# nextpyp/spr_pick

Measured on AMD Instinct MI355X. Metric: train_patches_per_sec, higher is better.
Workload: dtype f32; 1 GPU; BASELINE configs[1]: ssdn --noise_style gaussian --noise_value var, joint mode, 64x64 patches from 4 synthetic 1024x1024 micrographs, batch 32 per GPU, alpha 0.75, tau 0.01, Adam; fp32 MFMA convolutions (Winograd F(2x2,3x3) for the wide 3x3 layers); per_gpu_batch=32, global_batch=32, patch=64, parallelism=single GPU

## Files before the change

### include/sprk.h

```cpp
#ifndef SPRK_H
#define SPRK_H

#include <stddef.h>
#include <stdint.h>

#ifdef __cplusplus
extern "C" {
#endif

#define SPRK_OK 0
#define SPRK_EINVAL (-1)
#define SPRK_EWORKSPACE (-2)
#define SPRK_ELAUNCH (-3)

#define SPRK_ACT_NONE 0
#define SPRK_ACT_LEAKY 1
#define SPRK_ACT_RELU 2

typedef struct sprk_conv_geom {
    int32_t N, C1, C2, Hin, Win, up1;
    int32_t Cout, Hout, Wout;
    int32_t KH, KW, stride, dil, pad_top, pad_left;
    int32_t dtype;
} sprk_conv_geom;

#define SPRK_DT_F32 0
#define SPRK_DT_BF16 1
#define SPRK_DT_F16 2
#define SPRK_DT_MASK 0xff
#define SPRK_DT_FORCE 0x100
#define SPRK_DT_NAIVE 0x200
#define SPRK_DT_PIN 0x400
#define SPRK_DT_X16 0x8000
#define SPRK_DT_Y16 0x10000
#define SPRK_IO2(a, b) ((a) | ((b) << 4))
#define SPRK_IO3(a, b, c) ((a) | ((b) << 4) | ((c) << 8))

typedef struct sprk_conv_epilogue {
    const float *bias, *scale, *shift, *res;
    int32_t res_h, res_w, res_off;
    int32_t act;
    int32_t up2;
} sprk_conv_epilogue;

#define SPRK_ABI_VERSION 430
const char *sprk_last_error(void);
int sprk_version(void);
size_t sprk_struct_bytes(int which);
long sprk_launch_count(void);
long sprk_wino_launch_count(void);
long sprk_mask1x1_launch_count(void);
long sprk_conv16_launch_count(void);
long sprk_wgrad16_launch_count(void);

size_t sprk_conv2d_fwd_ws_bytes(const sprk_conv_geom *g);
int sprk_conv2d_fwd(const float *x, const float *x2, const float *w, float *y,
                    const sprk_conv_geom *g, const sprk_conv_epilogue *ep,
                    void *ws, size_t ws_bytes, void *stream);
size_t sprk_conv2d_bwd_data_ws_bytes(const sprk_conv_geom *g);
int sprk_conv2d_bwd_data(const float *gy, const float *w, float *gin, const sprk_conv_geom *g,
                         void *ws, size_t ws_bytes, void *stream);
size_t sprk_head1x1_fwd_ws_bytes(int K0, int N1);
int sprk_head1x1_fwd(const float *f, const float *w1, const float *b1, const float *w2, const float *b2,
                     const float *w3, const float *b3, float *out, int B, int K0, int N1, int N3, long HW, void *ws,
                     size_t ws_bytes, void *stream);

int sprk_head1x1_unrot_fwd(const float *d, const float *w1, const float *b1, const float *w2, const float *b2,
                           const float *w3, const float *b3, float *out, int B, int C, int P, int N3, void *ws,
                           size_t ws_bytes, void *stream);

int sprk_conv2d_bwd_data_masked(const float *gy, const float *w, float *gin, const sprk_conv_geom *g,
                                const float *mask_y, int mask_act, void *ws, size_t ws_bytes, void *stream);
int sprk_conv2d_bwd_data_mask_fused(const sprk_conv_geom *g);
int sprk_conv2d_storage16(const sprk_conv_geom *g, const sprk_conv_epilogue *ep);
size_t sprk_conv2d_bwd_weight_ws_bytes(const sprk_conv_geom *g);
int sprk_conv2d_bwd_weight(const float *x, const float *x2, const float *gy, float *gw,
                           const sprk_conv_geom *g, void *ws, size_t ws_bytes, void *stream);
#define SPRK_VARIANT_INTS 24
#define SPRK_STAGE_NONE (-2)
#define SPRK_STAGE_REFUSED (-1)
#define SPRK_STAGE_DIRECT 0
#define SPRK_STAGE_STEM 1
#define SPRK_STAGE_16BIT 2
#define SPRK_STAGE_WINOGRAD 3
#define SPRK_STAGE_MASK1X1 4
#define SPRK_STAGE_MFMA 5
int sprk_conv2d_variant(int which, const sprk_conv_geom *g, const sprk_conv_epilogue *ep, const void *x, const void *x2,
                        const void *y_or_gy, int32_t *out);
int sprk_conv2d_last_variant(int which, int32_t *out);

#define SPRK_DT_WPREP 0x800
#define SPRK_DT_WPREP_KIND(kind) (((kind) & 7) << 12)
#define SPRK_DT_WPREP_KIND_OF(dtype) (((dtype) >> 12) & 7)
typedef struct sprk_wprep_item {
    const float *w;
    void *dst;
    int32_t kind, blocks;
    int32_t p[12];
} sprk_wprep_item;
int sprk_conv2d_fwd_wprep(const float *w, const sprk_conv_geom *g, const sprk_conv_epilogue *ep, void *ws,
                          size_t ws_bytes, sprk_wprep_item *item);
int sprk_conv2d_bwd_data_wprep(const float *w, const sprk_conv_geom *g, void *ws, size_t ws_bytes, sprk_wprep_item *item);
int sprk_prepare_weights(const sprk_wprep_item *items, int n, void *stream);

size_t sprk_act_bwd_ws_bytes(int N, int C, int HW);
int sprk_act_bwd(const void *gy, const void *y, void *gpre, float *gbias, int act,
                 int N, int C, int H, int W, int up2, long g_image_stride, int io,
                 void *ws, size_t ws_bytes, void *stream);
#define SPRK_RED_NONE 0
#define SPRK_RED_ROWS 1
#define SPRK_RED_COLS 2
#define SPRK_RED_WGRAD 3
typedef struct sprk_reduce_item {
    const float *src;
    float *dst;
    int kind, parts, n, K, Cout, CoutP;
} sprk_reduce_item;
int sprk_conv2d_bwd_weight_partial(const float *x, const float *x2, const float *gy, float *gw,
                                   const sprk_conv_geom *g, void *ws, size_t ws_bytes,
                                   sprk_reduce_item *item, void *stream);
int sprk_act_bwd_partial(const void *gy, const void *y, void *gpre, float *gbias, int act,
                         int N, int C, int H, int W, int up2, long g_image_stride, int io,
                         void *ws, size_t ws_bytes, sprk_reduce_item *item, void *stream);
int sprk_reduce_items(const sprk_reduce_item *items, int n, void *stream);

int sprk_concat_up_bwd(const float *gin, float *ga, float *gb, int N, int C1, int C2, int H, int W,
                       int up1, void *stream);

int sprk_shift_maxpool2_fwd(const void *x, void *y, int NC, int H, int W, int shift, int io, void *stream);
int sprk_shift_maxpool2_bwd(const void *gy, const void *x, void *gx, int NC, int H, int W, int shift, int act,
                            int io, void *stream);
int sprk_rot4_stack_fwd(const float *x, float *y, int B, int C, int P, void *stream);
int sprk_rot4_stack_bwd(const float *gy, float *gx, int B, int C, int P, void *stream);
int sprk_unrot4_shift_concat_fwd(const void *d, void *f, int B, int C, int P, int io, void *stream);
int sprk_unrot4_shift_concat_bwd(const void *gf, void *gd, int B, int C, int P, int io, void *stream);
int sprk_unrot_act_bwd_eligible(int B, int C, int P, int act);
int sprk_conv2d_fwd_unrot_eligible(const sprk_conv_geom *g, const sprk_conv_epilogue *ep);
int sprk_conv2d_fwd_unrot(const float *x, const float *x2, const float *w, float *f, const sprk_conv_geom *g,
                          const sprk_conv_epilogue *ep, void *ws, size_t ws_bytes, void *stream);
// ... 105 lines not shown
```

### spr_pick_amd/_lib.py

```python
import ctypes
import os

_HERE = os.path.dirname(os.path.abspath(__file__))
LIB_PATH = os.environ.get("SPRK_LIB") or os.path.join(_HERE, "libsprk.so")

ACT_NONE, ACT_LEAKY, ACT_RELU = 0, 1, 2
DT_F32, DT_BF16, DT_F16 = 0, 1, 2
DT_NAIVE = 0x200
DT_WPREP = 0x800
DT_X16, DT_Y16 = 0x8000, 0x10000
DT_PIN = 0x400
DT_FORCE = 0x100
DTYPES = {"f32": DT_F32, "fp32": DT_F32, "bf16": DT_BF16, "f16": DT_F16, "fp16": DT_F16,
          "bf16!": DT_BF16 | DT_FORCE, "f16!": DT_F16 | DT_FORCE}

c_f = ctypes.c_void_p
c_i = ctypes.c_int
c_vp = ctypes.c_void_p
c_sz = ctypes.c_size_t


class ConvGeom(ctypes.Structure):
    _fields_ = [(n, ctypes.c_int32) for n in
                ("N", "C1", "C2", "Hin", "Win", "up1", "Cout", "Hout", "Wout",
                 "KH", "KW", "stride", "dil", "pad_top", "pad_left", "dtype")]


class ConvEpilogue(ctypes.Structure):
    _fields_ = [("bias", c_vp), ("scale", c_vp), ("shift", c_vp), ("res", c_vp),
                ("res_h", ctypes.c_int32), ("res_w", ctypes.c_int32), ("res_off", ctypes.c_int32),
                ("act", ctypes.c_int32), ("up2", ctypes.c_int32)]


class AdamItem(ctypes.Structure):
    _fields_ = [("p", c_vp), ("g", c_vp), ("m", c_vp), ("v", c_vp), ("n", ctypes.c_long)]


class ReduceItem(ctypes.Structure):
    _fields_ = [("src", c_vp), ("dst", c_vp), ("kind", ctypes.c_int32), ("parts", ctypes.c_int32), ("n", ctypes.c_int32),
                ("K", ctypes.c_int32), ("Cout", ctypes.c_int32), ("CoutP", ctypes.c_int32)]


class WprepItem(ctypes.Structure):
    _fields_ = [("w", c_vp), ("dst", c_vp), ("kind", ctypes.c_int32), ("blocks", ctypes.c_int32), ("p", ctypes.c_int32 * 12)]


_SIGS = {
    "sprk_last_error": (ctypes.c_char_p, []),
    "sprk_version": (c_i, []),
    "sprk_struct_bytes": (c_sz, [c_i]),
    "sprk_launch_count": (ctypes.c_long, []),
    "sprk_wino_launch_count": (ctypes.c_long, []),
    "sprk_mask1x1_launch_count": (ctypes.c_long, []),
    "sprk_conv16_launch_count": (ctypes.c_long, []),
    "sprk_wgrad16_launch_count": (ctypes.c_long, []),
    "sprk_conv2d_fwd_ws_bytes": (c_sz, [ctypes.POINTER(ConvGeom)]),
    "sprk_conv2d_fwd": (c_i, [c_f, c_f, c_f, c_f, ctypes.POINTER(ConvGeom), ctypes.POINTER(ConvEpilogue), c_vp, c_sz, c_vp]),
    "sprk_conv2d_fwd_wprep": (c_i, [c_f, ctypes.POINTER(ConvGeom), ctypes.POINTER(ConvEpilogue), c_vp, c_sz, ctypes.POINTER(WprepItem)]),
    "sprk_conv2d_bwd_data_wprep": (c_i, [c_f, ctypes.POINTER(ConvGeom), c_vp, c_sz, ctypes.POINTER(WprepItem)]),
    "sprk_prepare_weights": (c_i, [ctypes.POINTER(WprepItem), c_i, c_vp]),
    "sprk_head1x1_fwd_ws_bytes": (c_sz, [c_i, c_i]),
    "sprk_head1x1_fwd": (c_i, [c_f, c_f, c_f, c_f, c_f, c_f, c_f, c_f, c_i, c_i, c_i, c_i, ctypes.c_long, c_vp, c_sz, c_vp]),
    "sprk_head1x1_unrot_fwd": (c_i, [c_f, c_f, c_f, c_f, c_f, c_f, c_f, c_f, c_i, c_i, c_i, c_i, c_vp, c_sz, c_vp]),
    "sprk_conv2d_bwd_data_ws_bytes": (c_sz, [ctypes.POINTER(ConvGeom)]),
    "sprk_conv2d_bwd_data": (c_i, [c_f, c_f, c_f, ctypes.POINTER(ConvGeom), c_vp, c_sz, c_vp]),
    "sprk_conv2d_bwd_data_masked": (c_i, [c_f, c_f, c_f, ctypes.POINTER(ConvGeom), c_f, c_i, c_vp, c_sz, c_vp]),
    "sprk_conv2d_bwd_weight_ws_bytes": (c_sz, [ctypes.POINTER(ConvGeom)]),
    "sprk_conv2d_storage16": (c_i, [ctypes.POINTER(ConvGeom), ctypes.POINTER(ConvEpilogue)]),
    "sprk_conv2d_bwd_weight": (c_i, [c_f, c_f, c_f, c_f, ctypes.POINTER(ConvGeom), c_vp, c_sz, c_vp]),
    "sprk_conv2d_bwd_weight_partial": (c_i, [c_f, c_f, c_f, c_f, ctypes.POINTER(ConvGeom), c_vp, c_sz, ctypes.POINTER(ReduceItem), c_vp]),
    "sprk_act_bwd_partial": (c_i, [c_f, c_f, c_f, c_f, c_i, c_i, c_i, c_i, c_i, c_i, ctypes.c_long, c_i, c_vp, c_sz, ctypes.POINTER(ReduceItem), c_vp]),
    "sprk_reduce_items": (c_i, [ctypes.POINTER(ReduceItem), c_i, c_vp]),
    "sprk_act_bwd_ws_bytes": (c_sz, [c_i, c_i, c_i]),
    "sprk_act_bwd": (c_i, [c_f, c_f, c_f, c_f, c_i, c_i, c_i, c_i, c_i, c_i, ctypes.c_long, c_i, c_vp, c_sz, c_vp]),
    "sprk_concat_up_bwd": (c_i, [c_f, c_f, c_f, c_i, c_i, c_i, c_i, c_i, c_i, c_vp]),
    "sprk_shift_maxpool2_fwd": (c_i, [c_f, c_f, c_i, c_i, c_i, c_i, c_i, c_vp]),
    "sprk_shift_maxpool2_bwd": (c_i, [c_f, c_f, c_f, c_i, c_i, c_i, c_i, c_i, c_i, c_vp]),
    "sprk_rot4_stack_fwd": (c_i, [c_f, c_f, c_i, c_i, c_i, c_vp]),
    "sprk_rot4_stack_bwd": (c_i, [c_f, c_f, c_i, c_i, c_i, c_vp]),
    "sprk_unrot4_shift_concat_fwd": (c_i, [c_f, c_f, c_i, c_i, c_i, c_i, c_vp]),
    "sprk_unrot4_shift_concat_bwd": (c_i, [c_f, c_f, c_i, c_i, c_i, c_i, c_vp]),
    "sprk_unrot_act_bwd_eligible": (c_i, [c_i, c_i, c_i, c_i]),
    "sprk_conv2d_fwd_unrot_eligible": (c_i, [ctypes.POINTER(ConvGeom), ctypes.POINTER(ConvEpilogue)]),
    "sprk_conv2d_bwd_data_mask_fused": (c_i, [ctypes.POINTER(ConvGeom)]),
    "sprk_conv2d_variant": (c_i, [c_i, ctypes.POINTER(ConvGeom), ctypes.POINTER(ConvEpilogue), c_vp, c_vp, c_vp,
                                  ctypes.POINTER(ctypes.c_int32)]),
    "sprk_conv2d_last_variant": (c_i, [c_i, ctypes.POINTER(ctypes.c_int32)]),
    "sprk_conv2d_fwd_unrot": (c_i, [c_f, c_f, c_f, c_f, ctypes.POINTER(ConvGeom), ctypes.POINTER(ConvEpilogue), c_vp, c_sz, c_vp]),
    "sprk_unrot_act_bwd": (c_i, [c_f, c_f, c_f, c_f, c_i, c_i, c_i, c_i, c_vp, c_sz, ctypes.POINTER(ReduceItem), c_vp]),
    "sprk_bn_ws_bytes": (c_sz, [c_i, c_i, c_i, c_i]),
    "sprk_bn_train_fwd": (c_i, [c_f, c_f, c_f, c_f, c_f, c_f, c_f, c_f, c_i, c_i, c_i, c_i, ctypes.c_float, ctypes.c_float, c_i, c_vp, c_sz, c_vp]),
    "sprk_bn_eval_fwd": (c_i, [c_f, c_f, c_f, c_f, c_f, c_f, c_i, c_i, c_i, ctypes.c_float, c_i, c_vp]),
    "sprk_bn_train_bwd": (c_i, [c_f, c_f, c_f, c_f, c_f, c_f, c_f, c_f, c_f, c_i, c_i, c_i, c_i, c_i, c_vp, c_sz, c_vp]),
    "sprk_crop_add_fwd": (c_i, [c_f, c_f, c_f, ctypes.c_long, c_i, c_i, c_i, c_i, c_i, c_i, c_vp]),
    "sprk_crop_embed_bwd": (c_i, [c_f, c_f, ctypes.c_long, c_i, c_i, c_i, c_i, c_i, c_i, c_vp]),
    "sprk_noise_std_fwd": (c_i, [c_f, c_f, c_f, c_i, c_i, c_vp]),
    "sprk_noise_std_bwd": (c_i, [c_f, c_f, c_f, c_i, c_i, c_vp]),
    "sprk_joint_loss_fwd": (c_i, [c_f, c_f, c_f, c_f, c_f, c_f, c_i, c_i, c_i, c_i, ctypes.c_float, ctypes.c_float, c_vp]),
    "sprk_joint_loss_bwd": (c_i, [c_f, c_f, c_f, c_f, c_f, c_f, c_f, c_i, c_i, c_i, c_i, ctypes.c_float, ctypes.c_float, c_vp]),
    "sprk_reparam_fwd": (c_i, [c_f, c_f, c_f, c_i, c_i, c_vp]),
    "sprk_reparam_bwd": (c_i, [c_f, c_f, c_f, c_f, c_i, c_i, c_vp]),
    "sprk_adam_multi": (c_i, [c_vp, c_vp, c_i, c_i, c_f, c_f, c_f, ctypes.c_float, ctypes.c_float, ctypes.c_float, c_vp]),
    "sprk_adam_multi_skip": (c_i, [c_vp, c_vp, c_i, c_i, c_f, c_f, c_f, ctypes.c_float, ctypes.c_float, ctypes.c_float, c_vp, c_vp]),
    "sprk_unscale_check": (c_i, [c_f, ctypes.c_long, c_f, c_vp, c_vp]),
    "sprk_loss_scale_update": (c_i, [c_f, c_f, c_vp, c_vp, c_vp, c_vp, ctypes.c_float, ctypes.c_float, c_i, c_vp]),
    "sprk_pu_loss": (c_i, [c_f, c_f, c_f, c_i, ctypes.c_float, c_f, c_f, c_vp]),
# ... 63 lines not shown
```

### spr_pick_amd/csrc/conv.hip

```cpp
#include "common.h"
#include "conv16.h"
#include "mask1x1.h"
#include "wgrad16.h"
#include "wino.h"
#include "wprep_dev.h"

#include <cstdlib>

#include "conv_dev.h"
#include "io_dev.h"


namespace {

inline bool naive_of(const sprk_conv_geom *g) { return (g->dtype & SPRK_DT_NAIVE) != 0; }

constexpr int kZeroFloats = 256;
__device__ __attribute__((aligned(64))) float g_zero_block[kZeroFloats];

__device__ __forceinline__ void stage_planes(float *dst, const float *base, long imgStride, long cs, int nch, int N,
                                             int Hin, int Win, int Ws, int up, int vec, const float *zeros,
                                             const PlaneGeom &g, int n0, int iy0, int ixa, int lw, int lane) {
    const int imgElems = g.inRows * g.pitch;
    const int planeElems = g.NI * imgElems;
    const int per = vec ? 256 : 64;
    const int nGroups = (planeElems + per - 1) / per;
    const int nw = g.nw;
    const int gstart = g.deal ? 0 : lw, gstep = g.deal ? 1 : nw, cstep = g.deal ? nw : 1;
    for (int gi = gstart; gi < nGroups; gi += gstep) {
        const int e = vec ? gi * 256 + lane * 4 : gi * 64 + lane;
        const int il = fast_div(e, g.invImg);
        const int rem = e - il * imgElems;
        const int r = fast_div(rem, g.invPitch);
        const int j = rem - r * g.pitch;
        const int n = n0 + il, iy = iy0 + r, ix = ixa + j;
        const bool inb = e < planeElems;
        const bool ok = inb && n < N && (unsigned)iy < (unsigned)Hin && (unsigned)ix < (unsigned)Win;
        const int cl0 = g.deal ? (lw + nw - (gi % nw)) % nw : 0;
        const float *p = base + (long)n * imgStride + (up ? (long)(iy >> 1) * Ws + (ix >> 1) : (long)iy * Ws + ix) +
                         (long)cl0 * cs;
        long step = (long)cstep * cs;
        if (!ok) {
            p = zeros + lane * 4;
            step = 0;
        }
        float *d = dst + gi * per + cl0 * g.cplane;
        for (int cl = cl0; cl < nch; cl += cstep) {
            if (inb) {
                if (vec)
                    dma16(p, d);
                else
                    dma4(p, d);
            }
            p += step;
// ... 1427 lines not shown
#endif

int sprk_conv2d_storage16(const sprk_conv_geom *g, const sprk_conv_epilogue *ep) {
    if (!g || check_geom(g) != SPRK_OK) return 0;
    const int dt = g->dtype & SPRK_DT_MASK;
    if ((dt != SPRK_DT_BF16 && dt != SPRK_DT_F16) || naive_of(g) || g->stride != 1) return 0;
    sprk_conv_geom q = *g;
    q.dtype = (g->dtype & ~(SPRK_DT_WPREP | SPRK_DT_WPREP_KIND(7))) | SPRK_DT_X16 | SPRK_DT_Y16;
    int r = 0;
    if (sprk::conv16_kind(sprk::Corr(q, ep)) >= 2) r |= 1;
    if (sprk::conv16_kind(sprk::Corr(q)) >= 2) r |= 2;
    if (sprk::wgrad16_eligible(q)) r |= 4;
    return r;
}

static size_t corr_ws_bytes(const sprk::Corr &c) {
    FwdPlan p;
    if (!plan_fwd(c, &p)) return 0;
    size_t need = p.wsBytes;
    if (sprk::wino_eligible(c)) need = std::max(need, sprk::wino_ws_bytes(c));
    if (c.dt() != SPRK_DT_F32) need = std::max(need, sprk::conv16_ws_bytes(c));
    return need;
}

size_t sprk_conv2d_fwd_ws_bytes(const sprk_conv_geom *g) {
    if (!g) return 0;
    size_t need = 0;
    for (int v = 0; v < 4; ++v) {
        sprk_conv_epilogue e = sprk::kNoEpilogue;
        e.up2 = v & 1;
        e.res = (v & 2) ? (const float *)g : nullptr;
        need = std::max(need, corr_ws_bytes(sprk::Corr(*g, &e)));
    }
    return need;
}

size_t sprk_conv2d_bwd_data_ws_bytes(const sprk_conv_geom *g) {
    return (g && g->stride == 1) ? corr_ws_bytes(sprk::Corr(*g)) : 0;
}

static int mask_in_place(float *gin, const float *mask_y, int mask_act, const sprk_conv_geom *g, hipStream_t s) {
    const int t = (g->dtype & SPRK_DT_Y16) ? (g->dtype & SPRK_DT_MASK) : 0;
    return sprk_act_bwd(gin, mask_y, gin, nullptr, mask_act, g->N, g->C1 + g->C2, g->Hin, g->Win, 0, 0, SPRK_IO3(t, t, t),
                        nullptr, 0, s);
}

static bool mask1x1_takes(const sprk_conv_geom *g, const sprk::Corr &c, const FwdPlan &p) {
    return g->KH == 1 && g->KW == 1 && g->stride == 1 && g->dil == 1 && g->pad_top == 0 && g->pad_left == 0 && !g->up1 &&
           g->C2 == 0 && g->Hin == g->Hout && g->Win == g->Wout && c.dt() == SPRK_DT_F32 && !c.x16() && !c.y16() &&
           ((long)g->Hin * g->Win) % 4 == 0 && (long)g->Hin * g->Win < (1L << 30) && p.MT >= 2 &&
           sprk::mask1x1_steps(g->Cout, p.CK) > 0;
}

static FwdVariant fwd_route(bool bwd, const sprk_conv_geom *g, const sprk_conv_epilogue *ep, const void *x, const void *x2,
                            const void *y, const void *mask_y, FwdPlan *p, bool unrot = false) {
    FwdVariant v{};
    if (naive_of(g) || (bwd && g->stride != 1)) {
        StemPlan sp;
        v.stage = (bwd && !naive_of(g) && plan_stem_bwd(g, &sp)) ? SPRK_STAGE_STEM : SPRK_STAGE_DIRECT;
        return v;
    }
    const sprk::Corr c = bwd ? sprk::Corr(*g) : sprk::Corr(*g, ep);
    if (c.dt() != SPRK_DT_F32 && sprk::conv16_eligible(c)) {
        v.stage = SPRK_STAGE_16BIT;
    } else if (c.dtype & (SPRK_DT_X16 | SPRK_DT_Y16)) {
        v.stage = SPRK_STAGE_REFUSED;
    } else if (sprk::wino_eligible(c)) {
        v.stage = SPRK_STAGE_WINOGRAD;
        v.wino = sprk::wino_variant(c, mask_y != nullptr, unrot ? g->N / 4 : 0);
    } else if (!plan_fwd(c, p)) {
        v.stage = SPRK_STAGE_REFUSED;
    } else {
        v = fwd_variant(c, *p, x, x2, y);
        v.stage = (bwd && mask_y && mask1x1_takes(g, c, *p) && aligned16(x) && aligned16(y) && aligned16(mask_y))
                      ? SPRK_STAGE_MASK1X1
                      : SPRK_STAGE_MFMA;
    }
    return v;
}

static int conv_dispatch(bool bwd, const float *x, const float *x2, const float *w, float *y, const sprk_conv_geom *g,
                         const sprk_conv_epilogue *ep, const float *mask_y, int mask_act, void *ws, size_t ws_bytes,
                         void *stream, bool unrot = false) {
    const char *who = bwd ? "conv2d_bwd_data" : unrot ? "conv2d_fwd_unrot" : "conv2d_fwd";
    if (int rc = check_geom(g)) return rc;
    SPRK_REQUIRE(!unrot || sprk_conv2d_fwd_unrot_eligible(g, ep), "conv2d_fwd_unrot: no kernel with an un-rotated store for this layer");
    SPRK_REQUIRE(x && w && y, "%s: null tensor", who);
    if (bwd) {
        SPRK_REQUIRE(mask_act == SPRK_ACT_NONE || (mask_y && !g->up1), "conv2d_bwd_data: mask needs the saved input, no upsampling");
        if (mask_act == SPRK_ACT_NONE) mask_y = nullptr;
    } else {
        SPRK_REQUIRE(g->C2 == 0 || x2, "conv2d_fwd: C2 > 0 but x2 is null");
        SPRK_REQUIRE(!ep || !ep->scale || ep->shift, "conv2d_fwd: scale without shift");
    }
    hipStream_t s = (hipStream_t)stream;
    auto masked = [&](int rc) { return (rc || !mask_y) ? rc : mask_in_place(y, mask_y, mask_act, g, s); };

    FwdPlan p;
    const FwdVariant v = fwd_route(bwd, g, ep, x, x2, y, mask_y, &p, unrot);
    if (!sprk::wprep_describing()) t_last_fwd[bwd ? 1 : 0] = v;

    if (v.stage == SPRK_STAGE_DIRECT || v.stage == SPRK_STAGE_STEM) {
        if (sprk::wprep_describing()) return SPRK_OK;
        if (bwd) {
            DirectArgs a{nullptr, nullptr, w, x, y, *g, sprk::kNoEpilogue};
            StemPlan sp;
            if (v.stage == SPRK_STAGE_STEM && plan_stem_bwd(g, &sp)) {
                hipLaunchKernelGGL(conv_bwd_data_stem_kernel, dim3(g->N * sp.tilesX * sp.tilesY), dim3(kStemTW * kStemTH),
                                   sp.ldsBytes, s, a, sp.wr, sp.wc, sp.tilesX, sp.tilesY);
                return masked(sprk::check_launch("conv_bwd_data_stem"));
            }
            const long total = (long)g->N * (g->C1 + g->C2) * g->Hin * g->Win;
            hipLaunchKernelGGL(conv_bwd_data_direct_kernel, dim3(sprk::ew_blocks(total)), dim3(256), 0, s, a);
            return masked(sprk::check_launch("conv_bwd_data_direct"));
        }
        DirectArgs a{x, x2, w, nullptr, y, *g, ep ? *ep : sprk::kNoEpilogue};
        const long total = (long)g->N * g->Cout * g->Hout * g->Wout;
        hipLaunchKernelGGL(conv_fwd_direct_kernel, dim3(sprk::ew_blocks(total)), dim3(256), 0, s, a);
        return sprk::check_launch("conv_fwd_direct");
    }
    const sprk::Corr c = bwd ? sprk::Corr(*g) : sprk::Corr(*g, ep);

    if (v.stage == SPRK_STAGE_16BIT) return masked(sprk::conv16_run(c, x, x2, w, y, ws, ws_bytes, s));
    if (int rc = check_storage32(who, c.dtype)) return rc;

    if (v.stage == SPRK_STAGE_WINOGRAD) {
        if (int rc = sprk::check_ws(who, ws, ws_bytes, sprk::wino_ws_bytes(c))) return rc;
        if (int rc = sprk::wino_conv(c, v.wino, x, x2, w, y, (float *)ws, mask_y, mask_act, s)) return rc;
        return sprk::check_launch(bwd ? "wino_conv(bwd_data)" : "wino_conv");
    }
    SPRK_REQUIRE(!unrot, "conv2d_fwd_unrot: the call left the Winograd stage");

    SPRK_REQUIRE(v.stage != SPRK_STAGE_REFUSED, "%s: geometry does not fit LDS", who);
    if (int rc = sprk::check_ws(who, ws, ws_bytes, p.wsBytes)) return rc;
    float *wsf = (float *)ws;
    if (int rc = transform_weights(w, wsf, g->Cout, g->C1 + g->C2, g->KH * g->KW, c.taps, p, s)) return rc;
    if (v.stage == SPRK_STAGE_MASK1X1) {
        const sprk::Mask1x1Call m{x, wsf + kZeroFloats, mask_y, y, g->N, g->Cout, g->C1, g->Hin * g->Win,
                                  p.CK, p.R4, p.rows, p.ldw, p.NT, p.nblkN, mask_act};
        if (int rc = sprk::mask1x1_run(m, s)) return rc;
        return sprk::check_launch("mask1x1(bwd_data)");
    }
    const ConvArgs a = conv_args(c, p, v, x, x2, wsf, y);
    const int kclass = (v.MT == 4 && v.NT == 6) ? 0 : 2;
    sprk::prof_begin(kclass, c.flops, s);
    if (int rc = launch_fwd(a, p, v, s)) return rc;
    sprk::prof_end(kclass, s);
    return masked(sprk::check_launch(bwd ? "conv_mfma(bwd_data)" : "conv_mfma"));
}

int sprk_conv2d_fwd(const float *x, const float *x2, const float *w, float *y, const sprk_conv_geom *g,
                    const sprk_conv_epilogue *ep, void *ws, size_t ws_bytes, void *stream) {
    sprk::WprepScope scope(nullptr, g ? g->dtype : 0);
    return scope.verify(conv_dispatch(false, x, x2, w, y, g, ep, nullptr, SPRK_ACT_NONE, ws, ws_bytes, stream));
}

int sprk_conv2d_fwd_unrot_eligible(const sprk_conv_geom *g, const sprk_conv_epilogue *ep) {
    if (!g || check_geom(g) || naive_of(g)) return 0;
    const sprk::Corr c(*g, ep);
    if (c.dt() != SPRK_DT_F32 || c.x16() || c.y16()) return 0;
    return sprk::wino_unrot_eligible(c) ? 1 : 0;
}

int sprk_conv2d_fwd_unrot(const float *x, const float *x2, const float *w, float *f, const sprk_conv_geom *g,
                          const sprk_conv_epilogue *ep, void *ws, size_t ws_bytes, void *stream) {
    sprk::WprepScope scope(nullptr, g ? g->dtype : 0);
    return scope.verify(conv_dispatch(false, x, x2, w, f, g, ep, nullptr, SPRK_ACT_NONE, ws, ws_bytes, stream, true));
}

int sprk_conv2d_fwd_wprep(const float *w, const sprk_conv_geom *g, const sprk_conv_epilogue *ep, void *ws,
                          size_t ws_bytes, sprk_wprep_item *item) {
    SPRK_REQUIRE(item && w && ws, "conv2d_fwd_wprep: null argument");
    *item = sprk_wprep_item{};
    sprk::WprepScope scope(item, 0);
    const float *dummy = (const float *)ws;
    const int rc = conv_dispatch(false, dummy, g && g->C2 ? dummy : nullptr, w, (float *)ws, g, ep, nullptr, SPRK_ACT_NONE,
                                 ws, ws_bytes, nullptr);
    return rc == sprk::kWprepDescribed ? (int)SPRK_OK : rc;
}

int sprk_conv2d_bwd_data(const float *gy, const float *w, float *gin, const sprk_conv_geom *g, void *ws,
                         size_t ws_bytes, void *stream) {
    return sprk_conv2d_bwd_data_masked(gy, w, gin, g, nullptr, SPRK_ACT_NONE, ws, ws_bytes, stream);
}

int sprk_conv2d_bwd_data_masked(const float *gy, const float *w, float *gin, const sprk_conv_geom *g,
                                const float *mask_y, int mask_act, void *ws, size_t ws_bytes, void *stream) {
    sprk::WprepScope scope(nullptr, g ? g->dtype : 0);
    return scope.verify(conv_dispatch(true, gy, nullptr, w, gin, g, nullptr, mask_y, mask_act, ws, ws_bytes, stream));
}

int sprk_conv2d_bwd_data_mask_fused(const sprk_conv_geom *g) {
    if (!g || check_geom(g) != SPRK_OK || naive_of(g) || g->stride != 1 || g->up1) return 0;
    const sprk::Corr c(*g);
// ... 248 lines not shown
```

### spr_pick_amd/csrc/core.hip

```cpp
#include "common.h"
#include "wprep_dev.h"
#include "conv16.h"
#include "wgrad16.h"

#include <mutex>
#include <tuple>
#include <vector>

namespace sprk {

static thread_local char t_error[512] = "";
std::atomic<long> g_launches{0}, g_wino_launches{0}, g_mask1x1_launches{0};

void set_error(const char *fmt, ...) {
    va_list ap;
    va_start(ap, fmt);
    vsnprintf(t_error, sizeof(t_error), fmt, ap);
    va_end(ap);
}

constexpr int kMaxDev = 64;
int num_cus() {
    static std::atomic<int> cus[kMaxDev];
    int dev = 0;
    if (hipGetDevice(&dev) != hipSuccess || dev < 0 || dev >= kMaxDev) return 256;
    int v = cus[dev].load(std::memory_order_relaxed);
    if (v == 0) {
        if (hipDeviceGetAttribute(&v, hipDeviceAttributeMultiprocessorCount, dev) != hipSuccess || v <= 0) v = 256;
        cus[dev].store(v, std::memory_order_relaxed);
    }
    return v;
}

int lds_optin(const void *kernel, size_t bytes, const char *what) {
    if (bytes <= 64 * 1024) return SPRK_OK;
    static std::mutex mu;
    static std::vector<std::tuple<int, const void *, size_t>> done;
    int dev = 0;
    (void)hipGetDevice(&dev);
    std::lock_guard<std::mutex> lk(mu);
    for (auto &d : done)
        if (std::get<0>(d) == dev && std::get<1>(d) == kernel && std::get<2>(d) >= bytes) return SPRK_OK;
    if (hipFuncSetAttribute(kernel, hipFuncAttributeMaxDynamicSharedMemorySize, (int)bytes) != hipSuccess) {
        set_error("%s: cannot reserve %zu bytes of LDS", what, bytes);
        return SPRK_ELAUNCH;
    }
    done.emplace_back(dev, kernel, bytes);
    return SPRK_OK;
}

struct ProfRec {
    hipEvent_t a, b;
    int kclass;
    double flops, bytes;
};
// ... 183 lines not shown
    t_wprep_expect = t_wprep_seen = 0;
}
int WprepScope::verify(int rc) const {
    if (rc != SPRK_OK || !t_wprep_skip || !t_wprep_expect || t_wprep_seen == t_wprep_expect) return rc;
    set_error("prepared weights: the workspace holds a transform of another kind than this call's kernel path reads");
    return SPRK_EINVAL;
}
bool wprep_describing() { return t_wprep_describe != nullptr; }
int wprep_site(const sprk_wprep_item &it, hipStream_t s) {
    if (t_wprep_describe) {
        *t_wprep_describe = it;
        return kWprepDescribed;
    }
    if (t_wprep_skip) {
        t_wprep_seen = it.kind;
        if (t_wprep_expect && it.kind != t_wprep_expect) {
            set_error("prepared weights: the workspace holds a transform of another kind than this call's kernel path reads");
            return SPRK_EINVAL;
        }
        return SPRK_OK;
    }
    return wprep_launch(&it, 1, s);
}

}

extern "C" {

int sprk_prepare_weights(const sprk_wprep_item *items, int n, void *stream) {
    SPRK_REQUIRE(n >= 0 && (n == 0 || items), "prepare_weights: bad arguments");
    return sprk::wprep_launch(items, n, (hipStream_t)stream);
}

int sprk_reduce_items(const sprk_reduce_item *items, int n, void *stream) {
    SPRK_REQUIRE(n >= 0 && (n == 0 || items), "reduce_items: bad arguments");
    return sprk::reduce_items(items, n, (hipStream_t)stream);
}

const char *sprk_last_error(void) { return sprk::t_error; }
int sprk_version(void) { return SPRK_ABI_VERSION; }
size_t sprk_struct_bytes(int which) {
    switch (which) {
    case 0: return sizeof(sprk_conv_geom);
    case 1: return sizeof(sprk_conv_epilogue);
    case 2: return sizeof(sprk_reduce_item);
    case 3: return sizeof(sprk_adam_item);
    case 4: return sizeof(sprk_wprep_item);
    default: return 0;
    }
}
long sprk_launch_count(void) { return sprk::g_launches.load(); }
long sprk_wino_launch_count(void) { return sprk::g_wino_launches.load(); }
long sprk_mask1x1_launch_count(void) { return sprk::g_mask1x1_launches.load(); }
long sprk_conv16_launch_count(void) { return sprk::conv16_launches() + sprk::wgrad16_launches(); }
long sprk_wgrad16_launch_count(void) { return sprk::wgrad16_launches(); }

void sprk_prof_enable(int on) {
    std::lock_guard<std::mutex> lk(sprk::g_prof_mu);
    sprk::g_prof_mask = on;
}

int sprk_prof_collect(int kclass, long *launches, double *ms, double *flops) {
    return sprk_prof_collect_bytes(kclass, launches, ms, flops, nullptr);
}

int sprk_prof_collect_bytes(int kclass, long *launches, double *ms, double *flops, double *bytes) {
    std::lock_guard<std::mutex> lk(sprk::g_prof_mu);
    long n = 0;
    double t = 0.0, f = 0.0, by = 0.0;
    std::vector<sprk::ProfRec> keep;
    for (auto &r : sprk::g_recs) {
        if (r.kclass != kclass) {
            keep.push_back(r);
            continue;
        }
        float dt = 0.f;
        if (hipEventSynchronize(r.b) == hipSuccess && hipEventElapsedTime(&dt, r.a, r.b) == hipSuccess) {
            ++n;
            t += dt;
            f += r.flops;
            by += r.bytes;
        }
        sprk::g_pool.push_back({r.a, r.b});
    }
    sprk::g_recs.swap(keep);
    if (launches) *launches = n;
    if (ms) *ms = t;
    if (flops) *flops = f;
    if (bytes) *bytes = by;
    return SPRK_OK;
}

}
```

Before: 1977 patches/s.

## Add persistent double-buffered MFMA GEMM kernel for wide 1x1 convolutions

Adds a dedicated persistent GEMM kernel for f32 1x1 stride-1 convolutions with K>=192. It uses 256-pixel tiles, double-buffered buffer-DMA loads into LDS, up to two 96-channel output slabs per block and XCD-aware tile ordering, with bias/scale/activation fused into the store. Forward and unmasked backward-data calls are routed to it instead of the generic conv MFMA kernel. The aim is better operand reuse and overlap of loads with compute on the wide head layers, at the cost of a new code path and extra LDS use.

```diff
diff --git a/include/sprk.h b/include/sprk.h
--- a/include/sprk.h
+++ b/include/sprk.h
@@ -50,6 +50,8 @@
 long sprk_launch_count(void);
 long sprk_wino_launch_count(void);
 long sprk_mask1x1_launch_count(void);
+long sprk_gemm1x1_launch_count(void);
+void sprk_gemm1x1_enable(int on);
 long sprk_conv16_launch_count(void);
 long sprk_wgrad16_launch_count(void);
 
@@ -85,6 +87,7 @@
 #define SPRK_STAGE_WINOGRAD 3
 #define SPRK_STAGE_MASK1X1 4
 #define SPRK_STAGE_MFMA 5
+#define SPRK_STAGE_GEMM1X1 6
 int sprk_conv2d_variant(int which, const sprk_conv_geom *g, const sprk_conv_epilogue *ep, const void *x, const void *x2,
                         const void *y_or_gy, int32_t *out);
 int sprk_conv2d_last_variant(int which, int32_t *out);
diff --git a/scratch/head_gemm_bench.py b/scratch/head_gemm_bench.py
--- /dev/null
+++ b/scratch/head_gemm_bench.py
@@ -0,0 +1,68 @@
+import ctypes
+import statistics
+import sys
+
+import torch
+
+from spr_pick_amd import _lib, ops
+
+reps = int(sys.argv[1]) if len(sys.argv) > 1 else 10
+shapes = sys.argv[2] if len(sys.argv) > 2 else "main"
+L = _lib.lib()
+S = torch.ops.sprk
+dev = torch.device("cuda:0")
+have = "sprk_gemm1x1_enable" in _lib.EXPORTS
+g = torch.Generator().manual_seed(1)
+
+
+def timed(fn):
+    ts = []
+    out = None
+    for _ in range(reps):
+        a, b = torch.cuda.Event(enable_timing=True), torch.cuda.Event(enable_timing=True)
+        a.record()
+        out = fn()
+        b.record()
+        torch.cuda.synchronize()
+        ts.append(a.elapsed_time(b) * 1e3)
+    return out, ts
+
+
+def stage(which):
+    out = (ctypes.c_int32 * 24)()
+    L.sprk_conv2d_last_variant(which, out)
+    return out[0]
+
+
+CASES = {"main": [("fwd 384->384", 64, 384, 384, 64, False), ("fwd 384->96", 64, 384, 96, 64, False),
+                  ("bwd 384->384", 64, 384, 384, 64, True)],
+         "more": [("fwd 192->192", 64, 192, 192, 64, False), ("fwd 192->96", 64, 192, 96, 64, False),
+                  ("bwd 192->192", 64, 192, 192, 64, True), ("fwd 384->384 N32", 32, 384, 384, 64, False)]}
+
+for name, N, K, Cout, HW, bwd in CASES[shapes]:
+    x = torch.randn(N, K, HW, HW, generator=g).to(dev)
+    w = (torch.randn(Cout, K, 1, 1, generator=g) / K ** 0.5).to(dev)
+    b = torch.randn(Cout, generator=g).to(dev)
+    if bwd:
+        xin = torch.empty(N, Cout, HW, HW, device=dev)
+        wl = (torch.randn(K, Cout, 1, 1, generator=g) / K ** 0.5).to(dev)
+        geom = ops.make_geom(xin, None, wl, False, 1, 1, (0, 0, 0, 0))
+        fn = lambda: S.conv2d_bwd_data(x, wl, ops.geom_list(geom), None, ops.ACT_NONE, None)
+    else:
+        geom = ops.make_geom(x, None, w, False, 1, 1, (0, 0, 0, 0))
+        fn = lambda: ops.conv2d_forward(x, None, w, geom, bias=b, act=ops.ACT_LEAKY)
+    res = {}
+    for on in ((0, 1) if have else (None,)):
+        if on is not None:
+            L.sprk_gemm1x1_enable(on)
+        fn()
+        torch.cuda.synchronize()
+        out, ts = timed(fn)
+        res[on] = out
+        print("%-18s switch %-4s stage %d  median %.1f us  min %.1f  max %.1f  (%.1f TF at median)" % (
+            name, on, stage(1 if bwd else 0), statistics.median(ts), min(ts), max(ts),
+            2.0 * N * HW * HW * K * Cout / statistics.median(ts) * 1e-6), flush=True)
+    if have:
+        print("    on == off: %s" % torch.equal(res[0], res[1]), flush=True)
+    del x, w, res, out
+    torch.cuda.empty_cache()
diff --git a/scratch/kernel_csv_summary.py b/scratch/kernel_csv_summary.py
--- /dev/null
+++ b/scratch/kernel_csv_summary.py
@@ -0,0 +1,36 @@
+import csv
+import glob
+import os
+import re
+import sys
+from collections import defaultdict
+
+d, want = sys.argv[1], (sys.argv[2] if len(sys.argv) > 2 else "conv_mfma_kernel<4, 6|gemm1x1|mask1x1")
+pat = re.compile(want)
+
+
+def short(n):
+    n = re.sub(r"\(anonymous namespace\)::", "", n)
+    n = re.sub(r"^void ", "", n)
+    return n.split("(")[0][:60]
+
+
+for f in sorted(glob.glob(os.path.join(d, "**", "*kernel_trace.csv"), recursive=True)):
+    agg = defaultdict(list)
+    for r in csv.DictReader(open(f)):
+        k = short(r["Kernel_Name"])
+        if pat.search(k):
+            agg[(k, r.get("Grid_Size_X", ""), r.get("Grid_Size_Y", ""))].append((int(r["End_Timestamp"]) - int(r["Start_Timestamp"])) / 1e3)
+    for k, v in sorted(agg.items()):
+        v2 = sorted(v)
+        print("TRACE %-50s grid %s,%s  n %d  median %.1f us  min %.1f  mean %.1f" % (k[0], k[1], k[2], len(v), v2[len(v2) // 2], v2[0], sum(v) / len(v)))
+for f in sorted(glob.glob(os.path.join(d, "**", "*counter_collection.csv"), recursive=True)):
+    agg = defaultdict(lambda: defaultdict(list))
+    for r in csv.DictReader(open(f)):
+        k = short(r["Kernel_Name"])
+        if pat.search(k):
+            agg[(k, r.get("Grid_Size", ""), r.get("VGPR_Count", ""), r.get("Accum_VGPR_Count", ""), r.get("LDS_Block_Size", ""), r.get("Scratch_Size", ""))][r["Counter_Name"]].append(float(r["Counter_Value"]))
+    for k, cs in sorted(agg.items()):
+        print("PMC %-50s grid %s vgpr %s agpr %s lds %s scratch %s" % k)
+        for c, v in sorted(cs.items()):
+            print("      %-28s mean %.6g  (n %d)" % (c, sum(v) / len(v), len(v)))
diff --git a/spr_pick_amd/_lib.py b/spr_pick_amd/_lib.py
--- a/spr_pick_amd/_lib.py
+++ b/spr_pick_amd/_lib.py
@@ -52,6 +52,8 @@
     "sprk_launch_count": (ctypes.c_long, []),
     "sprk_wino_launch_count": (ctypes.c_long, []),
     "sprk_mask1x1_launch_count": (ctypes.c_long, []),
+    "sprk_gemm1x1_launch_count": (ctypes.c_long, []),
+    "sprk_gemm1x1_enable": (None, [c_i]),
     "sprk_conv16_launch_count": (ctypes.c_long, []),
     "sprk_wgrad16_launch_count": (ctypes.c_long, []),
     "sprk_conv2d_fwd_ws_bytes": (c_sz, [ctypes.POINTER(ConvGeom)]),
diff --git a/spr_pick_amd/csrc/conv.hip b/spr_pick_amd/csrc/conv.hip
--- a/spr_pick_amd/csrc/conv.hip
+++ b/spr_pick_amd/csrc/conv.hip
@@ -1,5 +1,6 @@
 #include "common.h"
 #include "conv16.h"
+#include "gemm1x1.h"
 #include "mask1x1.h"
 #include "wgrad16.h"
 #include "wino.h"
@@ -1533,6 +1534,13 @@
            sprk::mask1x1_steps(g->Cout, p.CK) > 0;
 }
 
+static bool gemm1x1_takes(const sprk::Corr &c, const FwdPlan &p) {
+    return sprk::g_gemm1x1_on.load(std::memory_order_relaxed) && c.KH == 1 && c.KW == 1 && c.stride == 1 && c.dil == 1 &&
+           c.padT == 0 && c.padL == 0 && !c.up1 && !c.mfma_only && c.C2 == 0 && !c.ep.up2 && !c.ep.res &&
+           c.Hin == c.Hout && c.Win == c.Wout && c.dt() == SPRK_DT_F32 && !c.x16() && !c.y16() && p.MT == 4 && p.NT == 6 &&
+           p.CK == 16 && p.R4 == 16 && p.ldw == sprk::kGemm1x1Ldw && sprk::gemm1x1_fits(c.N, c.C1, c.Hin * c.Win);
+}
+
 static FwdVariant fwd_route(bool bwd, const sprk_conv_geom *g, const sprk_conv_epilogue *ep, const void *x, const void *x2,
                             const void *y, const void *mask_y, FwdPlan *p, bool unrot = false) {
     FwdVariant v{};
@@ -1556,6 +1564,8 @@
         v.stage = (bwd && mask_y && mask1x1_takes(g, c, *p) && aligned16(x) && aligned16(y) && aligned16(mask_y))
                       ? SPRK_STAGE_MASK1X1
                       : SPRK_STAGE_MFMA;
+        if (v.stage == SPRK_STAGE_MFMA && !mask_y && !unrot && gemm1x1_takes(c, *p) && aligned16(x) && aligned16(y))
+            v.stage = SPRK_STAGE_GEMM1X1;
     }
     return v;
 }
@@ -1621,6 +1631,14 @@
                                   p.CK, p.R4, p.rows, p.ldw, p.NT, p.nblkN, mask_act};
         if (int rc = sprk::mask1x1_run(m, s)) return rc;
         return sprk::check_launch("mask1x1(bwd_data)");
+    }
+    if (v.stage == SPRK_STAGE_GEMM1X1) {
+        const sprk::Gemm1x1Call m{x, wsf + kZeroFloats, wsf, c.ep.bias, c.ep.scale, c.ep.shift, y, c.N, c.C1, c.Cout,
+                                  c.Hin * c.Win, p.rows, p.ldw, p.nblkN, c.ep.act};
+        sprk::prof_begin(0, c.flops, s);
+        if (int rc = sprk::gemm1x1_run(m, s)) return rc;
+        sprk::prof_end(0, s);
+        return sprk::check_launch(bwd ? "gemm1x1(bwd_data)" : "gemm1x1");
     }
     const ConvArgs a = conv_args(c, p, v, x, x2, wsf, y);
     const int kclass = (v.MT == 4 && v.NT == 6) ? 0 : 2;
diff --git a/spr_pick_amd/csrc/core.hip b/spr_pick_amd/csrc/core.hip
--- a/spr_pick_amd/csrc/core.hip
+++ b/spr_pick_amd/csrc/core.hip
@@ -1,6 +1,7 @@
 #include "common.h"
 #include "wprep_dev.h"
 #include "conv16.h"
+#include "gemm1x1.h"
 #include "wgrad16.h"
 
 #include <mutex>
@@ -290,6 +291,8 @@
 long sprk_launch_count(void) { return sprk::g_launches.load(); }
 long sprk_wino_launch_count(void) { return sprk::g_wino_launches.load(); }
 long sprk_mask1x1_launch_count(void) { return sprk::g_mask1x1_launches.load(); }
+long sprk_gemm1x1_launch_count(void) { return sprk::g_gemm1x1_launches.load(); }
+void sprk_gemm1x1_enable(int on) { sprk::g_gemm1x1_on.store(on ? 1 : 0); }
 long sprk_conv16_launch_count(void) { return sprk::conv16_launches() + sprk::wgrad16_launches(); }
 long sprk_wgrad16_launch_count(void) { return sprk::wgrad16_launches(); }
 
diff --git a/spr_pick_amd/csrc/gemm1x1.h b/spr_pick_amd/csrc/gemm1x1.h
--- /dev/null
+++ b/spr_pick_amd/csrc/gemm1x1.h
@@ -0,0 +1,25 @@
+#pragma once
+#include "common.h"
+
+namespace sprk {
+
+struct Gemm1x1Call {
+    const float *x, *wT, *zeros;
+    const float *bias, *scale, *shift;
+    float *y;
+    int N, K, Cn, HW;
+    int rows, ldw, nblkN;
+    int act;
+};
+
+constexpr int kGemm1x1MinK = 192;
+constexpr int kGemm1x1Ldw = 112;
+
+bool gemm1x1_fits(int N, int K, int HW);
+int gemm1x1_grid(int N, int HW, int nblkN);
+int gemm1x1_run(const Gemm1x1Call &c, hipStream_t s);
+
+extern std::atomic<long> g_gemm1x1_launches;
+extern std::atomic<int> g_gemm1x1_on;
+
+}
diff --git a/spr_pick_amd/csrc/gemm1x1.hip b/spr_pick_amd/csrc/gemm1x1.hip
--- /dev/null
+++ b/spr_pick_amd/csrc/gemm1x1.hip
@@ -0,0 +1,235 @@
+#include "gemm1x1.h"
+
+#include <type_traits>
+
+#include "conv_dev.h"
+
+namespace {
+
+constexpr int kTP = 256;
+constexpr int kXS = kTP + 16;
+constexpr int kKC = 32;
+constexpr int kLdw = sprk::kGemm1x1Ldw;
+constexpr int kWInstr = kKC * kLdw / 256;
+static_assert(kKC * kLdw % 256 == 0 && kXS % 32 == 16 && kLdw % 32 == 16, "LDS layout");
+
+struct G1Args {
+    const float *x, *wT, *scp, *shp;
+    float *y;
+    int N, K, Cn, HW;
+    int rows, nblkN;
+    int act, hasSc, hasSh;
+    int steps, nch, c0last;
+    int tilesPerImg, nTiles, nh, xcd;
+};
+
+template <int NB>
+__global__ __launch_bounds__(256) void gemm1x1_kernel(const G1Args a) {
+    extern __shared__ __attribute__((aligned(16))) float smem[];
+    constexpr int NTT = NB * 6;
+    constexpr int stageFloats = kKC * kXS + NB * kKC * kLdw;
+    const int tid = threadIdx.x, lane = tid & 63;
+    const int wave = __builtin_amdgcn_readfirstlane(tid >> 6);
+    const int l15 = lane & 15, lq = lane >> 4;
+    const int G = gridDim.x;
+
+    auto decode = [&](int r, int &t, int &h) {
+        const int b = blockIdx.x;
+        if (a.xcd) {
+            const int j = b >> 3;
+            h = j % a.nh;
+            t = r * (G / a.nh) + (j / a.nh) * 8 + (b & 7);
+        } else {
+            const int it = r * G + b;
+            t = it / a.nh;
+            h = it - t * a.nh;
+        }
+        t = __builtin_amdgcn_readfirstlane(t);
+        h = __builtin_amdgcn_readfirstlane(h);
+        return t < a.nTiles;
+    };
+    const rsrc_t wr = make_rsrc(a.wT);
+    auto issue = [&](int t, int h, int ci, int b) {
+        const int n = __builtin_amdgcn_readfirstlane(t / a.tilesPerImg), p0 = (t - n * a.tilesPerImg) * kTP;
+        float *xs = smem + b * stageFloats;
+        float *ws = xs + kKC * kXS;
+        const rsrc_t xr = make_rsrc(a.x + (long)n * a.K * a.HW);
+        const int xv = min(p0 + lane * 4, a.HW - 4) * 4;
+        const int r0 = ci * kKC;
+#pragma unroll
+        for (int i = 0; i < kKC / 4; ++i) {
+            const int r = r0 + wave + 4 * i;
+            const int ch = r < a.K ? r : a.c0last;
+            bdma16(xr, xv, ch * a.HW * 4, xs + (wave + 4 * i) * kXS);
+        }
+        const int valid = min(kKC, a.rows - r0) * kLdw * 4 - 16;
+#pragma unroll
+        for (int i0 = 0; i0 < NB * kWInstr; i0 += 4) {
+            const int i = min(i0 + wave, NB * kWInstr - 1);
+            const int nbi = i / kWInstr, ii = i - nbi * kWInstr;
+            const int nb = min(h * NB + nbi, a.nblkN - 1);
+            bdma16(wr, min(ii * 1024 + lane * 16, valid), (nb * a.rows + r0) * (kLdw * 4), ws + nbi * (kKC * kLdw) + ii * 256);
+        }
+    };
+    constexpr int kDmaPerWave = kKC / 4 + (NB * kWInstr + 3) / 4;
+
+    int t, h;
+    bool ok = decode(0, t, h);
+    if (!ok) return;
+    issue(t, h, 0, 0);
+    const int abase = lds_addr(smem) + (lq * kXS + wave * 64 + l15) * 4;
+    const int bbase = lds_addr(smem + kKC * kXS) + (lq * kLdw + l15) * 4;
+    int g = 0;
+    for (int r = 0; ok; ++r) {
+        int tn, hn;
+        const bool okn = decode(r + 1, tn, hn);
+        const int n = __builtin_amdgcn_readfirstlane(t / a.tilesPerImg), p0 = (t - n * a.tilesPerImg) * kTP;
+        const int pix = p0 + wave * 64 + lq * 4;
+        float vsc[NTT], vsh[NTT];
+#pragma unroll
+        for (int j = 0; j < NTT; ++j) {
+            const int idx = min(h * (NB * 96) + j * 16 + l15, a.Cn - 1);
+            vsc[j] = a.scp[a.hasSc ? idx : 0];
+            vsh[j] = a.shp[a.hasSh ? idx : 0];
+        }
+        f32x4 acc[4][NTT];
+#pragma unroll
+        for (int mt = 0; mt < 4; ++mt)
+#pragma unroll
+            for (int j = 0; j < NTT; ++j) acc[mt][j] = f32x4{0.f, 0.f, 0.f, 0.f};
+
+        for (int ci = 0; ci < a.nch; ++ci, ++g) {
+            if (ci > 0 || r == 0) asm volatile("s_waitcnt vmcnt(0)" ::: "memory");
+            lds_only_barrier();
+            const bool lastc = ci + 1 == a.nch;
+            const int nq = min(kKC / 4, a.steps - ci * (kKC / 4));
+            const int sa = abase + (g & 1) * (stageFloats * 4), sb = bbase + (g & 1) * (stageFloats * 4);
+            float a0[4], b0[NTT], a1[4], b1[NTT];
+            auto ld = [&](float (&av)[4], float (&bv)[NTT], int q) {
+                lds_cfp ap = lds_f(sa + q * (4 * kXS * 4));
+#pragma unroll
+                for (int mt = 0; mt < 4; ++mt) av[mt] = ap[16 * mt];
+                lds_cfp bp = lds_f(sb + q * (4 * kLdw * 4));
+#pragma unroll
+                for (int j = 0; j < NTT; ++j) bv[j] = bp[(j / 6) * (kKC * kLdw) + 16 * (j % 6)];
+            };
+            auto mm = [&](const float (&av)[4], const float (&bv)[NTT]) {
+#pragma unroll
+                for (int mt = 0; mt < 4; ++mt)
+#pragma unroll
+                    for (int j = 0; j < NTT; ++j)
+                        acc[mt][j] = __builtin_amdgcn_mfma_f32_16x16x4f32(av[mt], bv[j], acc[mt][j], 0, 0, 0);
+            };
+            const int last = nq - 1;
+            ld(a0, b0, 0);
+            ld(a1, b1, min(1, last));
+            {
+                const bool own = !lastc || !okn;
+                issue(own ? t : tn, own ? h : hn, lastc ? 0 : ci + 1, (g + 1) & 1);
+            }
+            mm(a0, b0);
+#pragma unroll
+            for (int i = 0; i < kDmaPerWave; ++i) {
+                __builtin_amdgcn_sched_group_barrier(0x008, 4 * NTT / kDmaPerWave, 0);
+                __builtin_amdgcn_sched_group_barrier(0x020, 1, 0);
+            }
+            for (int q = 1; q + 1 < nq; q += 2) {
+                ld(a0, b0, q + 1);
+                mm(a1, b1);
+                ld(a1, b1, min(q + 2, last));
+                mm(a0, b0);
+            }
+            if (!(nq & 1)) mm(a1, b1);
+        }
+        asm volatile("s_waitcnt vmcnt(0)" ::: "memory");
+#pragma unroll
+        for (int j = 0; j < NTT; ++j) asm volatile("" : "+v"(vsc[j]), "+v"(vsh[j]));
+        auto stores = [&](auto actc) {
+            constexpr int ACT = decltype(actc)::value;
+#pragma unroll
+            for (int j = 0; j < NTT; ++j) {
+                const int co = h * (NB * 96) + j * 16 + l15;
+                if (co >= a.Cn) continue;
+                const float sc = a.hasSc ? vsc[j] : 1.f, sh = vsh[j];
+                float *yc = a.y + ((long)n * a.Cn + co) * a.HW + pix;
+#pragma unroll
+                for (int mt = 0; mt < 4; ++mt) {
+                    if (pix + 16 * mt >= a.HW) continue;
+                    const f32x4 c = acc[mt][j];
+                    float v[4];
+#pragma unroll
+                    for (int e = 0; e < 4; ++e) v[e] = apply_act(c[e] * sc + sh, ACT);
+                    *reinterpret_cast<float4 *>(yc + 16 * mt) = make_float4(v[0], v[1], v[2], v[3]);
+                }
+            }
+        };
+        if (a.act == SPRK_ACT_LEAKY)
+            stores(std::integral_constant<int, SPRK_ACT_LEAKY>{});
+        else if (a.act == SPRK_ACT_RELU)
+            stores(std::integral_constant<int, SPRK_ACT_RELU>{});
+        else
+            stores(std::integral_constant<int, SPRK_ACT_NONE>{});
+        t = tn;
+        h = hn;
+        ok = okn;
+    }
+}
+
+inline int slabs_per_item(int nblkN) { return nblkN >= 2 ? 2 : 1; }
+
+template <int NB>
+int launch(const G1Args &a, int grid, hipStream_t s) {
+    const size_t lds = 2 * (size_t)(kKC * kXS + NB * kKC * kLdw) * sizeof(float);
+    if (int rc = sprk::lds_optin(gemm1x1_kernel<NB>, lds, "gemm1x1")) return rc;
+    hipLaunchKernelGGL(gemm1x1_kernel<NB>, dim3(grid), dim3(256), lds, s, a);
+    return SPRK_OK;
+}
+
+}
+
+namespace sprk {
+
+std::atomic<long> g_gemm1x1_launches{0};
+std::atomic<int> g_gemm1x1_on{1};
+
+bool gemm1x1_fits(int N, int K, int HW) {
+    return K >= kGemm1x1MinK && HW >= 4 && HW % 4 == 0 && (long)K * HW * 4 < (1L << 31) &&
+           (long)N * cdiv(HW, kTP) < (1L << 28);
+}
+
+int gemm1x1_grid(int N, int HW, int nblkN) {
+    const int nh = cdiv(nblkN, slabs_per_item(nblkN));
+    const long items = (long)N * cdiv(HW, kTP) * nh;
+    int G = (int)std::min<long>(items, num_cus());
+    if (G >= 8 * nh) G -= G % (8 * nh);
+    return std::max(G, 1);
+}
+
+int gemm1x1_run(const Gemm1x1Call &c, hipStream_t s) {
+    SPRK_REQUIRE(gemm1x1_fits(c.N, c.K, c.HW) && c.ldw == kLdw && c.rows == cdiv(c.K, 16) * 16 && c.nblkN >= 1 &&
+                     c.nblkN == cdiv(c.Cn, 96) && (long)c.nblkN * c.rows * kLdw * 4 < (1L << 31),
+                 "gemm1x1: call outside the kernel's limits");
+    const int NB = slabs_per_item(c.nblkN);
+    G1Args a{};
+    a.x = c.x; a.wT = c.wT; a.y = c.y;
+    a.scp = c.scale ? c.scale : c.zeros;
+    a.shp = c.scale ? c.shift : (c.bias ? c.bias : c.zeros);
+    a.hasSc = c.scale != nullptr;
+    a.hasSh = (c.scale || c.bias) ? 1 : 0;
+    a.N = c.N; a.K = c.K; a.Cn = c.Cn; a.HW = c.HW;
+    a.rows = c.rows; a.nblkN = c.nblkN;
+    a.act = c.act;
+    a.steps = cdiv(c.K, 4);
+    a.nch = cdiv(a.steps, kKC / 4);
+    a.c0last = (c.K - 1) / 16 * 16;
+    a.tilesPerImg = cdiv(c.HW, kTP);
+    a.nTiles = c.N * a.tilesPerImg;
+    a.nh = cdiv(c.nblkN, NB);
+    const int grid = gemm1x1_grid(c.N, c.HW, c.nblkN);
+    a.xcd = (grid % (8 * a.nh) == 0) ? 1 : 0;
+    if (int rc = NB == 2 ? launch<2>(a, grid, s) : launch<1>(a, grid, s)) return rc;
+    g_gemm1x1_launches.fetch_add(1, std::memory_order_relaxed);
+    return SPRK_OK;
+}
+
+}
```

Result: faster. 2000 patches/s (median of 6 runs) (+1.2%).
